# gotzmann/booster

Measured on AMD Instinct MI355X. Metric: decode tokens/sec Llama-3-8B Q4_K_M, higher is better.
Workload: dtype int8xint4/6 dot -> f32 (Q4_K/Q6_K weights x Q8_K activations), f16 KV; 1 GPU; Llama-3-8B Q4_K_M shapes (synthetic GGUF, random K-quant blocks), greedy batch-1 decode on 1xMI355X, 128-token prompt, n_ctx 2304, n_kv 133..2087; parallelism=single GPU, aql_runs=2, replay=AQL packets, fence scope NONE, own HSA queue (csrc/bamd_aql.h)

## Files before the change

### booster_amd/csrc/bamd_device.h

```cpp
#pragma once
#include <hip/hip_runtime.h>
#include <hip/hip_fp16.h>
#include <stdint.h>
#include <stdlib.h>
#include "bamd_formats.h"
#include "bamd_kernels.h"
#include "bamd_aql.h"

#define WAVE 64
#ifndef BAMD_SCHED_GROUP
#define BAMD_SCHED_GROUP 4
#endif

#ifdef BAMD_TIMING
#define TL_STAMP(tl, k) do { if ((tl) && (threadIdx.x & 63) == 0 && blockIdx.x < BAMD_TL_WG && blockIdx.y == 0) { const int w_ = (int) (threadIdx.x >> 6); \
        if (w_ == 0 || w_ == 7) (tl)[(size_t) blockIdx.x * BAMD_TL_WG_WORDS + (w_ ? 8 : 0) + (k)] = wall_clock64(); \
        if ((k) == 7 && w_ < 8) (tl)[(size_t) blockIdx.x * BAMD_TL_WG_WORDS + 16 + w_] = wall_clock64(); } } while (0)
#else
#define TL_STAMP(tl, k) do { } while (0)
#endif

__device__ __forceinline__ float h2f(uint32_t bits16) { return __half2float(__ushort_as_half((unsigned short) bits16)); }
__device__ __forceinline__ unsigned short f2h(float f) { return __half_as_ushort(__float2half_rn(f)); }
__device__ __forceinline__ int sdot4(uint32_t a, uint32_t b) { return __builtin_amdgcn_sdot4((int) a, (int) b, 0, false); }
// ... 117 lines not shown
    return __hiloint2double(__builtin_amdgcn_readlane(__double2hiint(v), lane), __builtin_amdgcn_readlane(__double2loint(v), lane));
}
__device__ __forceinline__ double wave_sum_f64(double s) {
    s += dpp_d<DPP_XOR1>(s); s += dpp_d<DPP_XOR2>(s); s += dpp_d<DPP_HALF_MIRROR>(s); s += dpp_d<DPP_MIRROR>(s);
    return ((readlane_d(s, 15) + readlane_d(s, 31)) + readlane_d(s, 47)) + readlane_d(s, 63);
}

#define BAMD_F64_GUARD_ULPS(n) (2 * (n) + 8)
__device__ __forceinline__ bool f32_rounding_safe(double v, int ulps) {
#ifdef BAMD_NO_F64_GUARD
    return true;
#endif
    if (v == 0.0) return true;
    const uint32_t hi = (uint32_t) __double2hiint(v), lo = (uint32_t) __double2loint(v);
    const uint32_t ex = (hi >> 20) & 0x7ffu;
    const int dist = (int) (lo & 0x1fffffffu) - 0x10000000;
    return ex >= 1023u - 126u && ex <= 1023u + 127u && (dist < 0 ? -dist : dist) > ulps;
}
__device__ __forceinline__ double seq_expsum8(const float * vals, int n) {
    double s = 0.0;
    for (int i = 0; i < n; i += 8) {
        const float a0 = vals[i] + vals[i + 4], a1 = vals[i + 1] + vals[i + 5], a2 = vals[i + 2] + vals[i + 6], a3 = vals[i + 3] + vals[i + 7];
        const float b0 = a0 + a2, b1 = a1 + a3;
        s += (double) (b0 + b1);
    }
    return s;
}

#define BAMD_ACT_BATCH 4
#ifndef BAMD_CEILING
#define BAMD_CEILING 0
#endif
#define BAMD_ACT_RED_OFF(nb) ((((size_t) (nb) * (256 + 32 + 4)) + 15) & ~(size_t) 15)
template <bool NORM>
struct ActPro {
    float4 v[BAMD_ACT_BATCH], w[BAMD_ACT_BATCH];
    int okmask;
    unsigned long long * tl = nullptr;

    template <int NB = BAMD_ACT_BATCH, int NWV = 0>
    __device__ __forceinline__ void issue(const float * __restrict__ x, const float * __restrict__ nw, int K, int i0, int bstride = 0, int blimit = 0) {
        const int lane = threadIdx.x & 63;
        if (bstride == 0) { bstride = NWV ? NWV : (int) (blockDim.x >> 6); blimit = K >> 8; }
        okmask = 0;
        const bamd_ik_rsrc rx = ik_rsrc(x);
#pragma unroll
        for (int b = 0; b < NB; ++b) {
            const int i = i0 + b * bstride;
            const bool ok = i < blimit;
            okmask |= ok ? 1 << b : 0;
            const int ic = ok ? i : blimit - 1;
            v[b] = ik_ld128f(rx, (uint32_t) lane * 16u, ic * 1024);
            if (NORM) w[b] = *(const float4 *) (nw + ic * 256 + lane * 4);
        }
    }

    template <int NB = BAMD_ACT_BATCH, int NWV = 0>
    __device__ __forceinline__ void quantize_batch(float scale, int K, int i0, uint32_t * q8, int * S, float * yd, int bstride = 0, int blimit = 0) {
        const int lane = threadIdx.x & 63;
        const int nwaves = bstride ? bstride : NWV ? NWV : (int) (blockDim.x >> 6), nb = bstride ? blimit : (K >> 8);
#if BAMD_CEILING & 1
#pragma unroll
        for (int b = 0; b < NB; ++b) {
            const int i = i0 + b * nwaves;
            if (i < nb) {
                const uint32_t packed = __float_as_uint(v[b].x) ^ (__float_as_uint(v[b].y) >> 8);
                q8[i * 64 + (lane & 7) * 8 + (lane >> 3)] = packed;
                if ((lane & 7) == 0) S[i * 8 + (lane >> 3)] = (int) (packed & 0xff);
                if (lane == 0) yd[i] = scale;
            }
        }
        return;
#endif
        uint32_t amaxb[NB];
#pragma unroll
        for (int b = 0; b < NB; ++b) {
            if (NORM) {
                v[b].x = (v[b].x * scale) * w[b].x; v[b].y = (v[b].y * scale) * w[b].y;
                v[b].z = (v[b].z * scale) * w[b].z; v[b].w = (v[b].w * scale) * w[b].w;
            }
            const float a = fmaxf(fmaxf(fmaxf(fabsf(v[b].x), fabsf(v[b].y)), fabsf(v[b].z)), fabsf(v[b].w));
            amaxb[b] = __float_as_uint(a);
        }
        uint32_t t[NB], wmax[NB];
#pragma unroll
        for (int b = 0; b < NB; ++b) t[b] = umax_(amaxb[b], (uint32_t) dpp_z<DPP_XOR1>((int) amaxb[b]));
#pragma unroll
        for (int b = 0; b < NB; ++b) t[b] = umax_(t[b], (uint32_t) dpp_z<DPP_XOR2>((int) t[b]));
#pragma unroll
        for (int b = 0; b < NB; ++b) t[b] = umax_(t[b], (uint32_t) dpp_z<DPP_HALF_MIRROR>((int) t[b]));
#pragma unroll
        for (int b = 0; b < NB; ++b) t[b] = umax_(t[b], (uint32_t) dpp_z<DPP_MIRROR>((int) t[b]));
#pragma unroll
        for (int b = 0; b < NB; ++b) t[b] = umax_(t[b], (uint32_t) __builtin_amdgcn_update_dpp(0, (int) t[b], 0x142, 0xa, 0xf, false));
#pragma unroll
        for (int b = 0; b < NB; ++b) t[b] = umax_(t[b], (uint32_t) __builtin_amdgcn_update_dpp(0, (int) t[b], 0x143, 0xc, 0xf, false));
#pragma unroll
        for (int b = 0; b < NB; ++b) wmax[b] = (uint32_t) __builtin_amdgcn_readlane((int) t[b], 63);
        float mine[NB];
#pragma unroll
        for (int b = 0; b < NB; ++b) {
            const float M = __uint_as_float(wmax[b]);
            const bool ex = fabsf(v[b].x) == M, ey = fabsf(v[b].y) == M, ez = fabsf(v[b].z) == M;
            float m = v[b].w;
            m = ez ? v[b].z : m; m = ey ? v[b].y : m; m = ex ? v[b].x : m;
            mine[b] = m;
        }
        int mxv = __float_as_int(1.0f);
#pragma unroll
        for (int b = 0; b < NB; ++b) {
            const unsigned long long who = __ballot(amaxb[b] == wmax[b]);
            const int first = __ffsll((long long) who) - 1;
            const int mxb = __builtin_amdgcn_readlane(__float_as_int(mine[b]), first);
            mxv = lane == b ? mxb : mxv;
        }
        const float isc = -127.f / __int_as_float(mxv);
        const float dd = 1.0f / isc;
#pragma unroll
        for (int b = 0; b < NB; ++b) {
            const int i = i0 + b * nwaves;
            if (i < nb) {
                const float iscale = __int_as_float(__builtin_amdgcn_readlane(__float_as_int(isc), b));
                const float d = __int_as_float(__builtin_amdgcn_readlane(__float_as_int(dd), b));
                const bool nz = wmax[b] != 0u;
                const float t0 = iscale * v[b].x + 12582912.f, t1 = iscale * v[b].y + 12582912.f;
                const float t2 = iscale * v[b].z + 12582912.f, t3 = iscale * v[b].w + 12582912.f;
                const uint32_t p01 = __builtin_amdgcn_perm(__float_as_uint(t1), __float_as_uint(t0), 0x0c0c0400u);
                const uint32_t p23 = __builtin_amdgcn_perm(__float_as_uint(t3), __float_as_uint(t2), 0x0c0c0400u);
                uint32_t packed = __builtin_amdgcn_perm(p23, p01, 0x05040100u);
                packed = nz ? packed : 0u;
                const int s4 = group8_sum(sdot4(packed, 0x01010101u));
                q8[i * 64 + (lane & 7) * 8 + (lane >> 3)] = packed;
                if ((lane & 7) == 0) S[i * 8 + (lane >> 3)] = s4;
                if (lane == 0) yd[i] = nz ? d : 0.f;
            }
        }
    }

    struct NoMid { __device__ __forceinline__ void operator()() const { } };
    template <bool SMALLK = false, typename MID = NoMid, int NB = BAMD_ACT_BATCH, int NWV = 0>
    __device__ __forceinline__ void finish(const float * __restrict__ x, const float * __restrict__ nw, float eps, int K,
                                           uint32_t * q8, int * S, float * yd, double * red, MID mid = MID()) {
        const int lane = threadIdx.x & 63, wave = wave_id(), nwaves = NWV ? NWV : (int) (blockDim.x >> 6), nb = K >> 8;
        const int step = nwaves * BAMD_ACT_BATCH;
        float scale = 1.0f;
#if BAMD_CEILING & 1
        if (NORM) { mid(); } else
#endif
        if (NORM) {
            double s = 0.0;
#pragma unroll
            for (int b = 0; b < NB; ++b) {
                if (okmask >> b & 1) { s += (double) (v[b].x * v[b].x); s += (double) (v[b].y * v[b].y); s += (double) (v[b].z * v[b].z); s += (double) (v[b].w * v[b].w); }
            }
            if (!SMALLK) for (int i0 = wave + step; i0 < nb; i0 += step) {
                ActPro<NORM> t; t.issue(x, nw, K, i0);
#pragma unroll
                for (int b = 0; b < BAMD_ACT_BATCH; ++b) {
                    if (t.okmask >> b & 1) { s += (double) (t.v[b].x * t.v[b].x); s += (double) (t.v[b].y * t.v[b].y); s += (double) (t.v[b].z * t.v[b].z); s += (double) (t.v[b].w * t.v[b].w); }
                }
            }
            s = wave_sum_f64(s);
            if (lane == 0) red[wave] = s;
            TL_STAMP(tl, 5);
            __syncthreads();
            mid();
            double tot = 0.0;
            for (int w2 = 0; w2 < nwaves; ++w2) tot += red[w2];
            double md = (K & (K - 1)) == 0 ? tot * (1.0 / (double) K) : tot / (double) K;
            float mean = (float) md;
            if (!f32_rounding_safe(md, BAMD_F64_GUARD_ULPS(K))) {
                __syncthreads();
                if (threadIdx.x == 0) {
                    double sq = 0.0;
                    for (int i = 0; i < K; ++i) { const float xv = ik_ld(x + i); sq += (double) (xv * xv); }
                    red[0] = sq;
                }
                __syncthreads();
                md = red[0] / (double) K;
                mean = (float) md;
            }
            scale = 1.0f / sqrtf(mean + eps);
        } else mid();
        quantize_batch<NB, NWV>(scale, K, wave, q8, S, yd);
        if (!SMALLK) for (int i0 = wave + step; i0 < nb; i0 += step) {
            ActPro<NORM> t; t.issue(x, nw, K, i0);
            t.quantize_batch(scale, K, i0, q8, S, yd);
        }
        TL_STAMP(tl, 6);
        __syncthreads();
    }
};

struct RowAcc { float acc, accm; };

struct RecQ4K { uint4 qs, hd; uint32_t mn47; };
struct RecQ5K { uint4 qs, hd; uint32_t qh, mn47; };
struct RecQ6K { uint4 ql; uint2 qh, sc; uint32_t d; };
struct RecQ3K { uint2 qs; uint32_t hm, sc0, sc1, sc2, d; };
struct RecQ2K { uint2 qs; uint4 sc; uint32_t dd; };

__device__ __forceinline__ void pin(uint32_t & x) { asm volatile("" : "+v"(x)); }
__device__ __forceinline__ void pin(uint2 & x) { pin(x.x); pin(x.y); }
__device__ __forceinline__ void pin(uint4 & x) { pin(x.x); pin(x.y); pin(x.z); pin(x.w); }
#if BAMD_XSCALES
__device__ __forceinline__ void pin_rec(RecQ4K & R) { pin(R.qs); pin(R.hd); pin(R.mn47); }
__device__ __forceinline__ void pin_rec(RecQ5K & R) { pin(R.qs); pin(R.hd); pin(R.qh); pin(R.mn47); }
#else
__device__ __forceinline__ void pin_rec(RecQ4K & R) { pin(R.qs); pin(R.hd); }
__device__ __forceinline__ void pin_rec(RecQ5K & R) { pin(R.qs); pin(R.hd); pin(R.qh); }
#endif
__device__ __forceinline__ void pin_rec(RecQ6K & R) { pin(R.ql); pin(R.qh); pin(R.sc); pin(R.d); }
__device__ __forceinline__ void pin_rec(RecQ3K & R) { pin(R.qs); pin(R.hm); pin(R.sc0); pin(R.sc1); pin(R.sc2); pin(R.d); }
__device__ __forceinline__ void pin_rec(RecQ2K & R) { pin(R.qs); pin(R.sc); pin(R.dd); }

typedef uint32_t u32x4_t __attribute__((ext_vector_type(4)));
typedef uint32_t u32x2_t __attribute__((ext_vector_type(2)));
// ... 39 lines not shown
    R.mn47 = 0u;
#endif
}
__device__ __forceinline__ void load_rec(RecQ5K & R, bamd_rsrc rs, int soff, int lane) {
    const uint32_t l = (uint32_t) lane;
    R.qs = bl128(rs, l * 16u, soff);
    R.qh = bl32(rs, 1024u + l * 4u, soff);
    R.hd = bl128(rs, 1280u + (l >> 3) * 16u, soff);
#if BAMD_XSCALES
    R.mn47 = bl32(rs, 1408u + (l >> 3) * 4u, soff);
#else
    R.mn47 = 0u;
#endif
}
__device__ __forceinline__ void load_rec(RecQ6K & R, bamd_rsrc rs, int soff, int lane) {
    const uint32_t l = (uint32_t) lane;
    R.ql = bl128(rs, l * 16u, soff);
    R.qh = bl64(rs, 1024u + l * 8u, soff);
    R.sc = bl64(rs, 1536u + (l >> 3) * 16u + ((l >> 2) & 1u) * 8u, soff);
    R.d  = bl16(rs, 1664u + (l >> 3) * 2u, soff);
}
__device__ __forceinline__ void load_rec(RecQ3K & R, bamd_rsrc rs, int soff, int lane) {
    const uint32_t l = (uint32_t) lane;
    R.qs = bl64(rs, l * 8u, soff);
    R.hm = bl32(rs, 512u + l * 4u, soff);
    R.sc0 = bl32(rs, 768u + (l >> 3) * 12u, soff); R.sc1 = bl32(rs, 772u + (l >> 3) * 12u, soff); R.sc2 = bl32(rs, 776u + (l >> 3) * 12u, soff);
    R.d  = bl16(rs, 864u + (l >> 3) * 2u, soff);
}
__device__ __forceinline__ void load_rec(RecQ2K & R, bamd_rsrc rs, int soff, int lane) {
    const uint32_t l = (uint32_t) lane;
    R.qs = bl64(rs, l * 8u, soff);
    R.sc = bl128(rs, 512u + (l >> 3) * 16u, soff);
    R.dd = bl32(rs, 640u + (l >> 3) * 4u, soff);
}
__device__ __forceinline__ void unpack_k4(const uint4 & hd, uint32_t & sc03, uint32_t & sc47, uint32_t & mn03, uint32_t & mn47) {
    const uint32_t u0 = hd.y, u1 = hd.z, u2 = hd.w;
    sc03 = u0 & 0x3f3f3f3fu; mn03 = u1 & 0x3f3f3f3fu;
    sc47 = (u2 & 0x0f0f0f0fu) | (((u0 >> 6) & 0x03030303u) << 4);
    mn47 = ((u2 >> 4) & 0x0f0f0f0fu) | (((u1 >> 6) & 0x03030303u) << 4);
}
#define BYTE(w, k) (int) (((w) >> (8 * (k))) & 0xffu)

struct Terms { float d, fs, dmin, pm; };

__device__ __forceinline__ Terms block_terms(const RecQ4K & R, int ci, int lane, const uint32_t * q8, const int * S, const float * yd) {
    const int e = lane & 7, l = e & 3;
    const float ydv = yd[ci];
    Terms T;
    T.d = ydv * h2f(R.hd.x & 0xffffu);
    T.dmin = (-ydv) * h2f(R.hd.x >> 16);
#if BAMD_XSCALES
    const uint32_t sc03 = R.hd.y, sc47 = R.hd.z, mn03 = R.hd.w, mn47 = R.mn47;
#else
    uint32_t sc03, sc47, mn03, mn47; unpack_k4(R.hd, sc03, sc47, mn03, mn47);
#endif
    const uint4 a0 = *(const uint4 *) (q8 + ci * 64 + e * 8), a1 = *(const uint4 *) (q8 + ci * 64 + e * 8 + 4);
    const uint32_t wq[8] = { R.qs.x & 0x0f0f0f0fu, (R.qs.x >> 4) & 0x0f0f0f0fu, R.qs.y & 0x0f0f0f0fu, (R.qs.y >> 4) & 0x0f0f0f0fu,
                             R.qs.z & 0x0f0f0f0fu, (R.qs.z >> 4) & 0x0f0f0f0fu, R.qs.w & 0x0f0f0f0fu, (R.qs.w >> 4) & 0x0f0f0f0fu };
    const uint32_t aq[8] = { a0.x, a0.y, a0.z, a0.w, a1.x, a1.y, a1.z, a1.w };
    const int sumi = dotscale8<false>(wq, aq, sc03, sc47);
    T.fs = (float) sumi;
    const uint32_t mw = (l < 2) ? mn03 : mn47;
    const int sh = (l & 1) * 16;
    const int ma = (int) ((mw >> sh) & 0xffu), mb = (int) ((mw >> (sh + 8)) & 0xffu);
    const int2 sp = *(const int2 *) (S + ci * 8 + 2 * l);
    T.pm = (float) (mul24(ma, sp.x) + mul24(mb, sp.y));
// ... 491 lines not shown
```

### booster_amd/csrc/bamd_matvec_core.h

```cpp
#pragma once
#include "bamd_device.h"
#include "bamd_mv_select.h"

template <int TYPE> struct RecOf;
template <> struct RecOf<BAMD_Q4_K> { typedef RecQ4K type; };
template <> struct RecOf<BAMD_Q5_K> { typedef RecQ5K type; };
template <> struct RecOf<BAMD_Q6_K> { typedef RecQ6K type; };
template <> struct RecOf<BAMD_Q3_K> { typedef RecQ3K type; };
template <> struct RecOf<BAMD_Q2_K> { typedef RecQ2K type; };

#define BAMD_NB1(NBW_) ((NBW_) < BAMD_ACT_BATCH ? (NBW_) : BAMD_ACT_BATCH)
#define BAMD_NB2(NBW_) ((NBW_) > BAMD_ACT_BATCH ? (NBW_) - BAMD_ACT_BATCH : 1)
#define BAMD_LEAD_PARAMS const float * x_, const float * nw_, const void * w0_, const void * w1_, int K_, float eps_
#define BAMD_LEAD_TAKE(a_) do { (a_).x = x_; (a_).normw = nw_; (a_).seg[0].w = w0_; (a_).seg[1].w = w1_; (a_).K = K_; (a_).eps = eps_; } while (0)
#define BAMD_LEAD_ARGS(a_) (a_).x, (a_).normw, (a_).seg[0].w, (a_).seg[1].w, (a_).K, (a_).eps
__device__ __forceinline__ ProArgs carve_lds(const bamd_mv_args & a, unsigned char * smem) {
    const int nb = a.K >> 8;
    ProArgs pa;
    pa.x = a.x; pa.nw = a.normw; pa.eps = a.eps; pa.K = a.K;
    pa.q8 = (uint32_t *) smem; pa.S = (int *) (pa.q8 + nb * 64); pa.yd = (float *) (pa.S + nb * 8);
    pa.tl = a.tl;
    pa.red = (double *) (smem + BAMD_ACT_RED_OFF(nb));
    return pa;
}


#define BAMD_EPI_HALF_GATE 16
#define BAMD_EPI_HALF_UP 17
template <int TYPE, int D, int EPI, int PRO, bool SMALLK = false, int NBP = BAMD_ACT_BATCH>
__device__ __forceinline__ void stream_segment(const uint8_t * __restrict__ wA, const uint8_t * __restrict__ wB, int nb,
                                               int first, int count, int stride, float * __restrict__ out,
                                               const float * __restrict__ res, const ProArgs & pa, ActPro<PRO == BAMD_PRO_NORM> & ap,
                                               bool issue_here, bool do_pro, unsigned long long & best, int nvalid, float * half_slot = nullptr, int * half_flag = nullptr) {
    typedef typename RecOf<TYPE>::type REC;
    constexpr int RECB = BAMD_RECB_OF(TYPE); static_assert(RECB > 0, "no wave-stream record for this type");
    constexpr bool PAIR = EPI == BAMD_EPI_SILU_MUL;
    constexpr int NPARTS = PAIR ? 2 : 1;
    const int lane = threadIdx.x & 63;
    const bamd_rsrc rsA = weight_rsrc(wA), rsB = PAIR ? weight_rsrc(wB) : rsA, rsN = null_rsrc(wA);
    const int rgb = nb * RECB;
    const int rg_step = stride * rgb;
    const int chunks = nb / D;
    if (issue_here) BAMD_PRO_ISSUE(ap, pa);
    REC ring[D];
    const int offA = count > 0 ? first * rgb : 0;
    const int fill_step = count > 0 ? RECB : 0;
#ifndef BAMD_RING_SPLIT
#define BAMD_RING_SPLIT 1
#endif
    constexpr bool RSPLIT = BAMD_RING_SPLIT && SMALLK && PRO == BAMD_PRO_NORM;
#pragma unroll
    for (int s = 0; s < (RSPLIT ? D / 2 : D); ++s) load_rec(ring[s], rsA, offA + s * fill_step, lane);
    TL_STAMP(pa.tl, 1);
    if (do_pro) {
        if (RSPLIT) {
            auto second_half = [&]() {
#pragma unroll
                for (int s = D / 2; s < D; ++s) load_rec(ring[s], rsA, offA + s * fill_step, lane);
            };
            BAMD_PRO_FINISH_NB_MID(ap, pa, second_half, NBP, 0);
        } else if (SMALLK) { auto nm = []() { }; BAMD_PRO_FINISH_NB_MID(ap, pa, nm, NBP, 0); }
        else BAMD_PRO_FINISH(ap, pa);
    } else if (RSPLIT) {
#pragma unroll
        for (int s = D / 2; s < D; ++s) load_rec(ring[s], rsA, offA + s * fill_step, lane);
    }
    TL_STAMP(pa.tl, 2);
    const uint32_t * q8 = pa.q8; const int * S = pa.S; const float * yd = pa.yd;
    for (int r = 0; r < count; ++r) {
        const int rg = first + r * stride;
        const int row = rg * 8 + (lane >> 3);
        const int rowoff = rg * rgb;
        float gate_val = 0.f;
#pragma unroll
        for (int part = 0; part < NPARTS; ++part) {
            const bool last = !(PAIR && part == 0) && r + 1 >= count;
            const bool after_b = (PAIR && part == 0) || (last && part == 1);
            const int after_off = (PAIR && part == 0) ? rowoff : (last ? rowoff + (nb - 1) * RECB : rowoff + rg_step);
            float resv = 0.f;
            if (EPI == BAMD_EPI_ADD && row < nvalid) resv = ik_ld(res + row);
            RowAcc A = { 0.f, 0.f };
            for (int c = 0; c < chunks; ++c) {
                const bool inrow = c + 1 < chunks;
                const bool tail = !inrow && last;
                const bamd_rsrc nrs = tail ? rsN : (inrow ? part == 1 : after_b) ? rsB : rsA;
                const int nxt = inrow ? rowoff + (c + 1) * (D * RECB) : after_off;
                const int step = (inrow || !last) ? RECB : 0;
#pragma unroll
                for (int s = 0; s < D; ++s) {
                    pin_rec(ring[s]);
                    const Terms T = block_terms(ring[s], c * D + s, lane, q8, S, yd);
                    chain_step<TYPE>(A, T.d, T.fs, T.dmin, T.pm);
                    load_rec(ring[s], nrs, nxt + s * step, lane);
                    if ((s & (BAMD_SCHED_GROUP - 1)) == BAMD_SCHED_GROUP - 1)
// ... 18 lines not shown
            } else if ((lane & 7) == 0 && row < nvalid) {
                float o = val;
                if (EPI == BAMD_EPI_ADD) o = val + resv;
                ik_st(out + row, o);
                if (EPI == BAMD_EPI_ARGMAX) { const unsigned long long k = argmax_key(o, row); best = k > best ? k : best; }
            }
        }
    }
}


template <int TYPE> __device__ __forceinline__ void hold_acc(RowAcc & A) {
    asm volatile("" : "+v"(A.acc));
    if (TYPE == BAMD_Q4_K || TYPE == BAMD_Q5_K) asm volatile("" : "+v"(A.accm));
}

template <int TYPE, int NBP, bool HELPER>
__device__ __forceinline__ void stream_pair_short(const uint8_t * __restrict__ wG, const uint8_t * __restrict__ wU, int rg0, int rg_stride, int j,
                                                  float * __restrict__ out, const ProArgs & pa, ActPro<true> & ap, float4 * park, int * flags, int nvalid) {
    typedef typename RecOf<TYPE>::type REC;
    constexpr int RECB = BAMD_RECB_OF(TYPE); static_assert(RECB > 0, "no wave-stream record for this type");
    constexpr int NB = 16, Q = NB / 4, CUT = NB - Q, D = 8, NREC = HELPER ? 3 * 2 * Q : 2 * CUT;
    static_assert(NREC % D == 0, "whole ring chunks");
    const int lane = threadIdx.x & 63;
    const bamd_rsrc rsG = weight_rsrc(wG), rsU = weight_rsrc(wU);
    const int rgb = NB * RECB;
#define BAMD_GU7_UP(i_)  (HELPER ? (((i_) % (2 * Q)) / Q) == 1 : ((i_) / CUT) == 1)
#define BAMD_GU7_SB(i_)  (HELPER ? CUT + ((i_) % Q) : (i_) % CUT)
#define BAMD_GU7_OFF(i_) ((HELPER ? rg0 + ((i_) / (2 * Q)) * rg_stride : rg0) * rgb + BAMD_GU7_SB(i_) * RECB)
    REC ring[D];
#pragma unroll
    for (int s = 0; s < D / 2; ++s) load_rec(ring[s], BAMD_GU7_UP(s) ? rsU : rsG, BAMD_GU7_OFF(s), lane);
    TL_STAMP(pa.tl, 1);
    auto second_half = [&]() {
#pragma unroll
        for (int s = D / 2; s < D; ++s) load_rec(ring[s], BAMD_GU7_UP(s) ? rsU : rsG, BAMD_GU7_OFF(s), lane);
    };
    BAMD_PRO_FINISH_NB_MID(ap, pa, second_half, NBP, 0);
    TL_STAMP(pa.tl, 2);
    const uint32_t * q8 = pa.q8; const int * S = pa.S; const float * yd = pa.yd;
    RowAcc Ag = { 0.f, 0.f }, Au = { 0.f, 0.f };
#pragma unroll
    for (int c = 0; c < NREC / D; ++c) {
#pragma unroll
        for (int s = 0; s < D; ++s) {
            const int i = c * D + s;
            pin_rec(ring[s]);
            const Terms T = block_terms(ring[s], BAMD_GU7_SB(i), lane, q8, S, yd);
            if (HELPER) park[((i / (2 * Q)) * 2 + (BAMD_GU7_UP(i) ? 1 : 0)) * Q * 64 + (i % Q) * 64 + lane] = make_float4(T.d, T.fs, T.dmin, T.pm);
            else if (BAMD_GU7_UP(i)) chain_step<TYPE>(Au, T.d, T.fs, T.dmin, T.pm);
            else chain_step<TYPE>(Ag, T.d, T.fs, T.dmin, T.pm);
            if (i + D < NREC) load_rec(ring[s], BAMD_GU7_UP(i + D) ? rsU : rsG, BAMD_GU7_OFF(i + D), lane);
            if (HELPER && (i % Q) == Q - 1) {
                __builtin_amdgcn_fence(__ATOMIC_RELEASE, "workgroup");
                if (lane == 0) __hip_atomic_store(flags + i / (2 * Q), (i % (2 * Q)) + 1, __ATOMIC_RELAXED, __HIP_MEMORY_SCOPE_WORKGROUP);
            }
            if ((s & (BAMD_SCHED_GROUP - 1)) == BAMD_SCHED_GROUP - 1) __builtin_amdgcn_sched_barrier(0);
        }
        if (c == 0) TL_STAMP(pa.tl, 3);
    }
    TL_STAMP(pa.tl, 4);
    if (!HELPER) {
        hold_acc<TYPE>(Ag); hold_acc<TYPE>(Au);
        const float4 * Pg = park + (j * 2 + 0) * Q * 64 + lane, * Pu = park + (j * 2 + 1) * Q * 64 + lane;
        auto wait_for = [&](const int need) {
            while (__hip_atomic_load(flags + j, __ATOMIC_RELAXED, __HIP_MEMORY_SCOPE_WORKGROUP) < need) __builtin_amdgcn_s_sleep(1);
            __builtin_amdgcn_fence(__ATOMIC_ACQUIRE, "workgroup");
        };
        float4 tg[Q], tu[Q];
        wait_for(Q);
#pragma unroll
// ... 43 lines not shown
    }
    int bbase = first * rgb + i0 * RECB;
    REC ring[D];
#ifndef BAMD_RING_SPLIT_B
#define BAMD_RING_SPLIT_B 1
#endif
#ifndef BAMD_RING_SPLIT_MIN
#define BAMD_RING_SPLIT_MIN 6
#endif
    constexpr bool RSPLIT = BAMD_RING_SPLIT_B && SMALLK && !UNEVEN && D >= BAMD_RING_SPLIT_MIN;
    constexpr int DH = RSPLIT ? D / 2 : D;
    auto ring_fill = [&](const int s0, const int s1) {
#pragma unroll
        for (int m = 0; m < M; ++m) {
            if (SMALLK || m < count) {
#pragma unroll
                for (int j = 0; j < NBW; ++j) {
                    const int sl = m * NBW + j;
                    if (sl >= s0 && sl < s1) load_rec(ring[sl], rs, bbase + m * rg_step + (UNEVEN && j >= n_w ? n_w - 1 : j) * RECB, lane);
                }
            }
        }
    };
    ring_fill(0, DH);
    TL_STAMP(pa.tl, 1);
    pre();
    if (do_pro) {
        if (OWN) {
            static_assert(NBW <= 2 * BAMD_ACT_BATCH, "own-slice prologue handles two batches");
            ap.template quantize_batch<BAMD_NB1(NBW)>(1.0f, pa.K, i0, pa.q8, pa.S, pa.yd, 1, i0 + n_w);
            if (RSPLIT) ring_fill(DH, D);
            if (NBW > BAMD_ACT_BATCH) ap2.template quantize_batch<BAMD_NB2(NBW)>(1.0f, pa.K, i0 + BAMD_ACT_BATCH, pa.q8, pa.S, pa.yd, 1, i0 + n_w);
        } else if (SMALLK && !UNEVEN) {
            auto second_half = [&]() { if (RSPLIT) ring_fill(DH, D); };
            BAMD_PRO_FINISH_NB_MID(ap, pa, second_half, BAMD_NB1(NBW), NWV);
        }
        else if (SMALLK) BAMD_PRO_FINISH_SMALLK(ap, pa);
        else BAMD_PRO_FINISH(ap, pa);
    } else if (RSPLIT) ring_fill(DH, D);
    TL_STAMP(pa.tl, 2);
    const uint32_t * q8 = pa.q8; const int * S = pa.S; const float * yd = pa.yd;
    for (int r0 = 0; r0 < (ONEB ? 1 : count); r0 += M) {
        const int nbatch = ONEB ? M : (count - r0 < M ? count - r0 : M);
        float * B0 = part0 + (NBUF == 2 ? (size_t) (batchctr & 1) * M * rg_floats : (size_t) 0);
        const int crow = (first + (r0 + (wave < nbatch ? wave : 0)) * stride) * 8 + r8;
        float resv = 0.f;
        if (EPI == BAMD_EPI_ADD && crow < nvalid) resv = ik_ld(res + crow);
#pragma unroll
        for (int m = 0; m < M; ++m) {
            if (m < nbatch) {
                float * Pf = B0 + (size_t) m * rg_floats;
                float4 * P = (float4 *) Pf;
#pragma unroll
                for (int j = 0; j < NBW; ++j) {
                    const int s = m * NBW + j;
                    const int ci = i0 + j;
                    pin_rec(ring[s]);
                    if (!UNEVEN || j < n_w) {
                        const Terms T = block_terms(ring[s], ci, lane, q8, S, yd);
                        if (COMPACT) {
                            float * rec = Pf + (size_t) ci * 144;
                            *(float2 *) (rec + lane * 2) = make_float2(T.fs, T.pm);
                            if ((lane & 7) == 0) *(float2 *) (rec + 128 + r8 * 2) = make_float2(T.d, T.dmin);
                        } else P[ci * 64 + lane] = make_float4(T.d, T.fs, T.dmin, T.pm);
                    }
#ifndef BAMD_SPLIT_UNCOND_REFILL
#define BAMD_SPLIT_UNCOND_REFILL 1
// ... 66 lines not shown
```

### booster_amd/csrc/bamd_matvec_fast_a.hip

```cpp
#include "bamd_matvec_core.h"

template <int TYPE0, int TYPE1, int PRO, int EPI, int NBP>
__global__ void __launch_bounds__(512) matvec_fast_kernel(BAMD_LEAD_PARAMS, bamd_mv_args a) {
    BAMD_LEAD_TAKE(a);
    extern __shared__ __attribute__((aligned(16))) unsigned char smem[];
    TL_STAMP(a.tl, 0);
    const int nb = a.K >> 8;
    const ProArgs pa = carve_lds(a, smem);
    ActPro<PRO == BAMD_PRO_NORM> ap;
    BAMD_PRO_ISSUE_NB(ap, pa, NBP, 0);
    const int wave = wave_id(), nwaves = blockDim.x >> 6;
    const int slot = blockIdx.x + gridDim.x * wave;
    const int stride = gridDim.x * nwaves;
    unsigned long long best = 0ull;
    constexpr bool PAIR = EPI == BAMD_EPI_SILU_MUL;
    const int nrg0 = a.seg[0].nrows >> 3;
    const int nv0 = a.seg[0].nvalid > 0 ? a.seg[0].nvalid : a.seg[0].nrows;
    if (TYPE1 == 0) {
        const int count = a.cnt_q + (slot < a.cnt_r ? 1 : 0);
        const uint8_t * wA = (const uint8_t *) a.seg[0].w;
        const uint8_t * wB = PAIR ? (const uint8_t *) a.seg[1].w : wA;
        stream_segment<TYPE0, 8, EPI, PRO, true, NBP>(wA, wB, nb, slot, count, stride, a.seg[0].out, a.res, pa, ap, false, true, best, nv0);
    } else {
        constexpr int T1 = TYPE1 == 0 ? TYPE0 : TYPE1;
        const int nrg1 = a.seg[1].nrows >> 3;
        const int nv1 = a.seg[1].nvalid > 0 ? a.seg[1].nvalid : a.seg[1].nrows;
        if (slot >= nrg0 && slot < nrg0 + nrg1) {
            const uint8_t * w1 = (const uint8_t *) a.seg[1].w;
            stream_segment<T1, 8, EPI, PRO, true, NBP>(w1, w1, nb, slot - nrg0, 1, stride, a.seg[1].out, a.res, pa, ap, false, true, best, nv1);
        } else {
            const uint8_t * w0 = (const uint8_t *) a.seg[0].w;
            stream_segment<TYPE0, 8, EPI, PRO, true, NBP>(w0, w0, nb, slot, slot < nrg0 ? 1 : 0, stride, a.seg[0].out, a.res, pa, ap, false, true, best, nv0);
        }
    }
    if (EPI == BAMD_EPI_ARGMAX) {
        for (int o = 32; o; o >>= 1) { const unsigned long long ob = __shfl_xor(best, o); best = ob > best ? ob : best; }
        __syncthreads();
        unsigned long long * wb = (unsigned long long *) smem;
        if ((threadIdx.x & 63) == 0) wb[wave] = best;
        __syncthreads();
        if (threadIdx.x == 0) {
            unsigned long long b = 0ull;
            for (int w = 0; w < nwaves; ++w) b = wb[w] > b ? wb[w] : b;
            if (b) atomicMax(a.best_key, b);
        }
    }
    TL_STAMP(a.tl, 7);
}

template <int TYPE, int NBP>
__global__ void __launch_bounds__(512) matvec_gateup7_kernel(BAMD_LEAD_PARAMS, bamd_mv_args a) {
    BAMD_LEAD_TAKE(a);
    extern __shared__ __attribute__((aligned(16))) unsigned char smem[];
    TL_STAMP(a.tl, 0);
    const int nb = a.K >> 8;
    const ProArgs pa = carve_lds(a, smem);
    ActPro<true> ap;
    BAMD_PRO_ISSUE_NB(ap, pa, NBP, 0);
    const int wave = wave_id(), grid = (int) gridDim.x, b = (int) blockIdx.x;
    float4 * park = (float4 *) (smem + mv_park_off(nb));
    int * flags = (int *) (smem + mv_park_off(nb) + mv_gu7_park_bytes(16));
    if (threadIdx.x < 4) flags[threadIdx.x] = 0;
    const uint8_t * wG = (const uint8_t *) a.seg[0].w, * wU = (const uint8_t *) a.seg[1].w;
    const int nv = a.seg[0].nvalid > 0 ? a.seg[0].nvalid : a.seg[0].nrows;
    unsigned long long best = 0ull;
    if (wave < 4) stream_segment<TYPE, 8, BAMD_EPI_SILU_MUL, BAMD_PRO_NORM, true, NBP>(wG, wU, nb, b + grid * wave, 1, grid * 8, a.seg[0].out, a.res, pa, ap, false, true, best, nv);
    else if (wave < 7) stream_pair_short<TYPE, NBP, false>(wG, wU, b + grid * wave, grid, wave - 4, a.seg[0].out, pa, ap, park, flags, nv);
    else stream_pair_short<TYPE, NBP, true>(wG, wU, b + grid * 4, grid, 0, a.seg[0].out, pa, ap, park, flags, nv);
    TL_STAMP(a.tl, 7);
}
static const bool g_gateup7 = env_flag("BAMD_GATEUP7", true);

template <int TYPE, int NBP>
__global__ void __launch_bounds__(512) matvec_gateup14_kernel(BAMD_LEAD_PARAMS, bamd_mv_args a) {
    BAMD_LEAD_TAKE(a);
    extern __shared__ __attribute__((aligned(16))) unsigned char smem[];
    TL_STAMP(a.tl, 0);
    const int nb = a.K >> 8;
    const ProArgs pa = carve_lds(a, smem);
    ActPro<true> ap;
    BAMD_PRO_ISSUE_NB(ap, pa, NBP, 0);
    const int wave = wave_id(), grid = (int) gridDim.x, b = (int) blockIdx.x;
    float * slots = (float *) (smem + mv_park_off(nb));
    int * flags = (int *) (slots + 16);
    if (threadIdx.x < 2) flags[threadIdx.x] = 0;
    const uint8_t * wG = (const uint8_t *) a.seg[0].w, * wU = (const uint8_t *) a.seg[1].w;
    const int nv = a.seg[0].nvalid > 0 ? a.seg[0].nvalid : a.seg[0].nrows;
    unsigned long long best = 0ull;
    if (wave < 4) stream_segment<TYPE, 8, BAMD_EPI_SILU_MUL, BAMD_PRO_NORM, true, NBP>(wG, wU, nb, b + grid * wave, 2, grid * 4, a.seg[0].out, a.res, pa, ap, false, true, best, nv);
    else {
        stream_segment<TYPE, 8, BAMD_EPI_SILU_MUL, BAMD_PRO_NORM, true, NBP>(wG, wU, nb, b + grid * (4 + wave), 1, grid, a.seg[0].out, a.res, pa, ap, false, true, best, nv);
        const int h = (wave - 4) >> 1;
        const int rg = b + grid * (12 + h);
        if (((wave - 4) & 1) == 0) stream_segment<TYPE, 8, BAMD_EPI_HALF_GATE, BAMD_PRO_NORM, true, NBP>(wG, wG, nb, rg, 1, grid, a.seg[0].out, a.res, pa, ap, false, false, best, nv, slots + 8 * h, flags + h);
        else                       stream_segment<TYPE, 8, BAMD_EPI_HALF_UP, BAMD_PRO_NORM, true, NBP>(wU, wU, nb, rg, 1, grid, a.seg[0].out, a.res, pa, ap, false, false, best, nv, slots + 8 * h, flags + h);
    }
    TL_STAMP(a.tl, 7);
}
static const bool g_gateup14 = env_flag("BAMD_GATEUP14", true);

template <int PRO, int EPI, int T0, int T1>
static void launch_fast_a_inst(const bamd_mv_args & a, int grid, hipStream_t s) {
    if ((a.K >> 8) <= 16) BAMD_LAUNCH((matvec_fast_kernel<T0, T1, PRO, EPI, 2>), dim3(grid), dim3(512), act_lds_bytes(a.K), s, BAMD_LEAD_ARGS(a), a);
    else                  BAMD_LAUNCH((matvec_fast_kernel<T0, T1, PRO, EPI, 4>), dim3(grid), dim3(512), act_lds_bytes(a.K), s, BAMD_LEAD_ARGS(a), a);
}
typedef pairs<cpair<BAMD_Q4_K, BAMD_Q5_K>, cpair<BAMD_Q4_K, BAMD_Q6_K>, cpair<BAMD_Q5_K, BAMD_Q4_K>, cpair<BAMD_Q5_K, BAMD_Q6_K>, cpair<BAMD_Q6_K, BAMD_Q4_K>,
              cpair<BAMD_Q6_K, BAMD_Q5_K>, cpair<BAMD_Q2_K, BAMD_Q3_K>> fast_a_pairs;
template <int PRO, int EPI>
static bool launch_fast_a_types(const bamd_mv_args & a, int t0, int t1, int grid, hipStream_t s) {
    if (t1 == 0) return with_kquant(t0, [&](auto T) -> bool { launch_fast_a_inst<PRO, EPI, decltype(T)::value, 0>(a, grid, s); return true; });
    if constexpr (PRO == BAMD_PRO_NORM && EPI == BAMD_EPI_STORE)
        return with_pair(fast_a_pairs(), t0, t1, [&](auto P) -> bool { launch_fast_a_inst<PRO, EPI, decltype(P)::a, decltype(P)::b>(a, grid, s); return true; });
    return false;
}
// ... 23 lines not shown
```

Baseline: 686.9 tokens/s.

## Interleave second-half ring weight loads across RMSnorm/quantize prologue stages

Splits the second half of the weight-record ring prefetch into per-field load parts and spreads them over named stage points in the activation norm and quantize prologue: the DPP reduction steps, the barrier, mean, scale, max reductions and the divide. Scheduling barriers pin each group of loads at its stage. The aim is to overlap weight memory issue with the prologue's latency-bound reduction chain instead of issuing all loads in one burst at the barrier. It also makes the wave count a compile-time constant (8) for the fast_a kernels. This costs more code complexity and register pressure, and it assumes 512-thread blocks.

```diff
diff --git a/booster_amd/csrc/bamd_device.h b/booster_amd/csrc/bamd_device.h
--- a/booster_amd/csrc/bamd_device.h
+++ b/booster_amd/csrc/bamd_device.h
@@ -173,6 +173,35 @@
 #define BAMD_CEILING 0
 #endif
 #define BAMD_ACT_RED_OFF(nb) ((((size_t) (nb) * (256 + 32 + 4)) + 15) & ~(size_t) 15)
+template <int N> struct StageC { static constexpr int value = N; };
+template <int LO, int HI, typename F> __device__ __forceinline__ void static_for(F && f) {
+    if constexpr (LO < HI) { f(StageC<LO>()); static_for<LO + 1, HI>(f); }
+}
+enum {
+    BAMD_ST_SQ = 0,
+    BAMD_ST_SQ1,
+    BAMD_ST_SQ2, BAMD_ST_SQ3, BAMD_ST_SQ4,
+    BAMD_ST_BAR,
+    BAMD_ST_RED,
+    BAMD_ST_MEAN,
+    BAMD_ST_SCALE,
+    BAMD_ST_NORM,
+    BAMD_ST_MAX1,
+    BAMD_ST_MAX2, BAMD_ST_MAX3, BAMD_ST_MAX4, BAMD_ST_MAX5, BAMD_ST_MAX6,
+    BAMD_ST_FIRST,
+    BAMD_ST_DIV,
+    BAMD_ST_END,
+    BAMD_ST_COUNT
+};
+template <typename MID, typename = void> struct MidStaged { static constexpr bool value = false; };
+template <typename MID> struct MidStaged<MID, decltype((*(MID *) nullptr)(StageC<0>()), void())> { static constexpr bool value = true; };
+template <int ST, typename MID> __device__ __forceinline__ void mid_at(MID & mid, int) {
+    if constexpr (MidStaged<MID>::value) mid(StageC<ST>());
+    else if constexpr (ST == BAMD_ST_BAR) mid();
+}
+template <int LO, int HI, typename MID> __device__ __forceinline__ void mid_span(MID & mid) {
+    static_for<LO, HI>([&](auto st) { mid_at<decltype(st)::value>(mid, 0); });
+}
 template <bool NORM>
 struct ActPro {
     float4 v[BAMD_ACT_BATCH], w[BAMD_ACT_BATCH];
@@ -196,11 +225,13 @@
         }
     }
 
-    template <int NB = BAMD_ACT_BATCH, int NWV = 0>
-    __device__ __forceinline__ void quantize_batch(float scale, int K, int i0, uint32_t * q8, int * S, float * yd, int bstride = 0, int blimit = 0) {
+    struct NoMid { __device__ __forceinline__ void operator()() const { } };
+    template <int NB = BAMD_ACT_BATCH, int NWV = 0, typename MID = NoMid>
+    __device__ __forceinline__ void quantize_batch(float scale, int K, int i0, uint32_t * q8, int * S, float * yd, int bstride = 0, int blimit = 0, MID mid = MID()) {
         const int lane = threadIdx.x & 63;
         const int nwaves = bstride ? bstride : NWV ? NWV : (int) (blockDim.x >> 6), nb = bstride ? blimit : (K >> 8);
 #if BAMD_CEILING & 1
+        mid_span<BAMD_ST_NORM, BAMD_ST_DIV + 1>(mid);
 #pragma unroll
         for (int b = 0; b < NB; ++b) {
             const int i = i0 + b * nwaves;
@@ -223,19 +254,26 @@
             const float a = fmaxf(fmaxf(fmaxf(fabsf(v[b].x), fabsf(v[b].y)), fabsf(v[b].z)), fabsf(v[b].w));
             amaxb[b] = __float_as_uint(a);
         }
+        mid_at<BAMD_ST_NORM>(mid, 0);
         uint32_t t[NB], wmax[NB];
 #pragma unroll
         for (int b = 0; b < NB; ++b) t[b] = umax_(amaxb[b], (uint32_t) dpp_z<DPP_XOR1>((int) amaxb[b]));
+        mid_at<BAMD_ST_MAX1>(mid, 0);
 #pragma unroll
         for (int b = 0; b < NB; ++b) t[b] = umax_(t[b], (uint32_t) dpp_z<DPP_XOR2>((int) t[b]));
+        mid_at<BAMD_ST_MAX2>(mid, 0);
 #pragma unroll
         for (int b = 0; b < NB; ++b) t[b] = umax_(t[b], (uint32_t) dpp_z<DPP_HALF_MIRROR>((int) t[b]));
+        mid_at<BAMD_ST_MAX3>(mid, 0);
 #pragma unroll
         for (int b = 0; b < NB; ++b) t[b] = umax_(t[b], (uint32_t) dpp_z<DPP_MIRROR>((int) t[b]));
+        mid_at<BAMD_ST_MAX4>(mid, 0);
 #pragma unroll
         for (int b = 0; b < NB; ++b) t[b] = umax_(t[b], (uint32_t) __builtin_amdgcn_update_dpp(0, (int) t[b], 0x142, 0xa, 0xf, false));
+        mid_at<BAMD_ST_MAX5>(mid, 0);
 #pragma unroll
         for (int b = 0; b < NB; ++b) t[b] = umax_(t[b], (uint32_t) __builtin_amdgcn_update_dpp(0, (int) t[b], 0x143, 0xc, 0xf, false));
+        mid_at<BAMD_ST_MAX6>(mid, 0);
 #pragma unroll
         for (int b = 0; b < NB; ++b) wmax[b] = (uint32_t) __builtin_amdgcn_readlane((int) t[b], 63);
         float mine[NB];
@@ -255,8 +293,10 @@
             const int mxb = __builtin_amdgcn_readlane(__float_as_int(mine[b]), first);
             mxv = lane == b ? mxb : mxv;
         }
+        mid_at<BAMD_ST_FIRST>(mid, 0);
         const float isc = -127.f / __int_as_float(mxv);
         const float dd = 1.0f / isc;
+        mid_at<BAMD_ST_DIV>(mid, 0);
 #pragma unroll
         for (int b = 0; b < NB; ++b) {
             const int i = i0 + b * nwaves;
@@ -278,7 +318,6 @@
         }
     }
 
-    struct NoMid { __device__ __forceinline__ void operator()() const { } };
     template <bool SMALLK = false, typename MID = NoMid, int NB = BAMD_ACT_BATCH, int NWV = 0>
     __device__ __forceinline__ void finish(const float * __restrict__ x, const float * __restrict__ nw, float eps, int K,
                                            uint32_t * q8, int * S, float * yd, double * red, MID mid = MID()) {
@@ -286,7 +325,7 @@
         const int step = nwaves * BAMD_ACT_BATCH;
         float scale = 1.0f;
 #if BAMD_CEILING & 1
-        if (NORM) { mid(); } else
+        if (NORM) { if constexpr (MidStaged<MID>::value) mid_span<BAMD_ST_SQ, BAMD_ST_SCALE + 1>(mid); else mid(); } else
 #endif
         if (NORM) {
             double s = 0.0;
@@ -301,13 +340,21 @@
                     if (t.okmask >> b & 1) { s += (double) (t.v[b].x * t.v[b].x); s += (double) (t.v[b].y * t.v[b].y); s += (double) (t.v[b].z * t.v[b].z); s += (double) (t.v[b].w * t.v[b].w); }
                 }
             }
-            s = wave_sum_f64(s);
+            if constexpr (MidStaged<MID>::value) {
+                mid_at<BAMD_ST_SQ>(mid, 0);
+                s += dpp_d<DPP_XOR1>(s);        mid_at<BAMD_ST_SQ1>(mid, 0);
+                s += dpp_d<DPP_XOR2>(s);        mid_at<BAMD_ST_SQ2>(mid, 0);
+                s += dpp_d<DPP_HALF_MIRROR>(s); mid_at<BAMD_ST_SQ3>(mid, 0);
+                s += dpp_d<DPP_MIRROR>(s);      mid_at<BAMD_ST_SQ4>(mid, 0);
+                s = ((readlane_d(s, 15) + readlane_d(s, 31)) + readlane_d(s, 47)) + readlane_d(s, 63);
+            } else s = wave_sum_f64(s);
             if (lane == 0) red[wave] = s;
             TL_STAMP(tl, 5);
             __syncthreads();
-            mid();
+            if constexpr (MidStaged<MID>::value) mid_at<BAMD_ST_BAR>(mid, 0); else mid();
             double tot = 0.0;
             for (int w2 = 0; w2 < nwaves; ++w2) tot += red[w2];
+            mid_at<BAMD_ST_RED>(mid, 0);
             double md = (K & (K - 1)) == 0 ? tot * (1.0 / (double) K) : tot / (double) K;
             float mean = (float) md;
             if (!f32_rounding_safe(md, BAMD_F64_GUARD_ULPS(K))) {
@@ -321,9 +368,14 @@
                 md = red[0] / (double) K;
                 mean = (float) md;
             }
+            mid_at<BAMD_ST_MEAN>(mid, 0);
             scale = 1.0f / sqrtf(mean + eps);
-        } else mid();
-        quantize_batch<NB, NWV>(scale, K, wave, q8, S, yd);
+            mid_at<BAMD_ST_SCALE>(mid, 0);
+        } else if constexpr (MidStaged<MID>::value) mid_span<BAMD_ST_SQ, BAMD_ST_SCALE + 1>(mid);
+        else mid();
+        if constexpr (MidStaged<MID>::value) quantize_batch<NB, NWV, MID &>(scale, K, wave, q8, S, yd, 0, 0, mid);
+        else quantize_batch<NB, NWV>(scale, K, wave, q8, S, yd);
+        mid_at<BAMD_ST_END>(mid, 0);
         if (!SMALLK) for (int i0 = wave + step; i0 < nb; i0 += step) {
             ActPro<NORM> t; t.issue(x, nw, K, i0);
             t.quantize_batch(scale, K, i0, q8, S, yd);
@@ -429,6 +481,55 @@
     R.qs = bl64(rs, l * 8u, soff);
     R.sc = bl128(rs, 512u + (l >> 3) * 16u, soff);
     R.dd = bl32(rs, 640u + (l >> 3) * 4u, soff);
+}
+template <typename REC> struct RecLoads;
+template <> struct RecLoads<RecQ4K> { static constexpr int value = BAMD_XSCALES ? 3 : 2; };
+template <> struct RecLoads<RecQ5K> { static constexpr int value = BAMD_XSCALES ? 4 : 3; };
+template <> struct RecLoads<RecQ6K> { static constexpr int value = 4; };
+template <> struct RecLoads<RecQ3K> { static constexpr int value = 6; };
+template <> struct RecLoads<RecQ2K> { static constexpr int value = 3; };
+template <int P> __device__ __forceinline__ void load_rec_part(RecQ4K & R, bamd_rsrc rs, int soff, int lane) {
+    const uint32_t l = (uint32_t) lane;
+    if (P == 0) R.qs = bl128(rs, l * 16u, soff);
+    if (P == 1) R.hd = bl128(rs, 1024u + (l >> 3) * 16u, soff);
+#if BAMD_XSCALES
+    if (P == 2) R.mn47 = bl32(rs, 1152u + (l >> 3) * 4u, soff);
+#else
+    if (P == 1) R.mn47 = 0u;
+#endif
+}
+template <int P> __device__ __forceinline__ void load_rec_part(RecQ5K & R, bamd_rsrc rs, int soff, int lane) {
+    const uint32_t l = (uint32_t) lane;
+    if (P == 0) R.qs = bl128(rs, l * 16u, soff);
+    if (P == 1) R.qh = bl32(rs, 1024u + l * 4u, soff);
+    if (P == 2) R.hd = bl128(rs, 1280u + (l >> 3) * 16u, soff);
+#if BAMD_XSCALES
+    if (P == 3) R.mn47 = bl32(rs, 1408u + (l >> 3) * 4u, soff);
+#else
+    if (P == 2) R.mn47 = 0u;
+#endif
+}
+template <int P> __device__ __forceinline__ void load_rec_part(RecQ6K & R, bamd_rsrc rs, int soff, int lane) {
+    const uint32_t l = (uint32_t) lane;
+    if (P == 0) R.ql = bl128(rs, l * 16u, soff);
+    if (P == 1) R.qh = bl64(rs, 1024u + l * 8u, soff);
+    if (P == 2) R.sc = bl64(rs, 1536u + (l >> 3) * 16u + ((l >> 2) & 1u) * 8u, soff);
+    if (P == 3) R.d  = bl16(rs, 1664u + (l >> 3) * 2u, soff);
+}
+template <int P> __device__ __forceinline__ void load_rec_part(RecQ3K & R, bamd_rsrc rs, int soff, int lane) {
+    const uint32_t l = (uint32_t) lane;
+    if (P == 0) R.qs = bl64(rs, l * 8u, soff);
+    if (P == 1) R.hm = bl32(rs, 512u + l * 4u, soff);
+    if (P == 2) R.sc0 = bl32(rs, 768u + (l >> 3) * 12u, soff);
+    if (P == 3) R.sc1 = bl32(rs, 772u + (l >> 3) * 12u, soff);
+    if (P == 4) R.sc2 = bl32(rs, 776u + (l >> 3) * 12u, soff);
+    if (P == 5) R.d  = bl16(rs, 864u + (l >> 3) * 2u, soff);
+}
+template <int P> __device__ __forceinline__ void load_rec_part(RecQ2K & R, bamd_rsrc rs, int soff, int lane) {
+    const uint32_t l = (uint32_t) lane;
+    if (P == 0) R.qs = bl64(rs, l * 8u, soff);
+    if (P == 1) R.sc = bl128(rs, 512u + (l >> 3) * 16u, soff);
+    if (P == 2) R.dd = bl32(rs, 640u + (l >> 3) * 4u, soff);
 }
 __device__ __forceinline__ void unpack_k4(const uint4 & hd, uint32_t & sc03, uint32_t & sc47, uint32_t & mn03, uint32_t & mn47) {
     const uint32_t u0 = hd.y, u1 = hd.z, u2 = hd.w;
diff --git a/booster_amd/csrc/bamd_matvec_core.h b/booster_amd/csrc/bamd_matvec_core.h
--- a/booster_amd/csrc/bamd_matvec_core.h
+++ b/booster_amd/csrc/bamd_matvec_core.h
@@ -24,6 +24,29 @@
     return pa;
 }
 
+
+#ifndef BAMD_RING_DRIP
+#define BAMD_RING_DRIP 1
+#endif
+#ifndef BAMD_RING_DRIP_B
+#define BAMD_RING_DRIP_B 0
+#endif
+#ifndef BAMD_PRO_NWV_A
+#define BAMD_PRO_NWV_A 8
+#endif
+template <int MODE, int ST, int NL, typename ONE> __device__ __forceinline__ void drip_stage(ONE && one) {
+    constexpr int FIRST = MODE == 2 ? BAMD_ST_SQ1 : MODE == 3 ? BAMD_ST_END : BAMD_ST_BAR, LAST = MODE == 3 ? BAMD_ST_END : BAMD_ST_DIV;
+    constexpr int NS = LAST - FIRST + 1, PER = (NL + NS - 1) / NS, k = ST - FIRST;
+    static_assert(NS >= 1 && PER * NS >= NL, "every request has a stage point");
+    if constexpr (k >= 0 && k < NS) {
+        constexpr int lo = k * PER < NL ? k * PER : NL, hi = (k + 1) * PER < NL ? (k + 1) * PER : NL;
+        if constexpr (lo < hi) {
+            __builtin_amdgcn_sched_barrier(0);
+            static_for<lo, hi>(one);
+            __builtin_amdgcn_sched_barrier(0);
+        }
+    }
+}
 
 #define BAMD_EPI_HALF_GATE 16
 #define BAMD_EPI_HALF_UP 17
@@ -54,12 +77,22 @@
     TL_STAMP(pa.tl, 1);
     if (do_pro) {
         if (RSPLIT) {
+#if BAMD_RING_DRIP
+            constexpr int LPR = RecLoads<REC>::value;
+            auto second_half = [&](auto st) {
+                drip_stage<BAMD_RING_DRIP, decltype(st)::value, (D - D / 2) * LPR>([&](auto n) {
+                    constexpr int s = D / 2 + decltype(n)::value / LPR;
+                    load_rec_part<decltype(n)::value % LPR>(ring[s], rsA, offA + s * fill_step, lane);
+                });
+            };
+#else
             auto second_half = [&]() {
 #pragma unroll
                 for (int s = D / 2; s < D; ++s) load_rec(ring[s], rsA, offA + s * fill_step, lane);
             };
-            BAMD_PRO_FINISH_NB_MID(ap, pa, second_half, NBP, 0);
-        } else if (SMALLK) { auto nm = []() { }; BAMD_PRO_FINISH_NB_MID(ap, pa, nm, NBP, 0); }
+#endif
+            BAMD_PRO_FINISH_NB_MID(ap, pa, second_half, NBP, BAMD_PRO_NWV_A);
+        } else if (SMALLK) { auto nm = []() { }; BAMD_PRO_FINISH_NB_MID(ap, pa, nm, NBP, BAMD_PRO_NWV_A); }
         else BAMD_PRO_FINISH(ap, pa);
     } else if (RSPLIT) {
 #pragma unroll
@@ -144,11 +177,21 @@
 #pragma unroll
     for (int s = 0; s < D / 2; ++s) load_rec(ring[s], BAMD_GU7_UP(s) ? rsU : rsG, BAMD_GU7_OFF(s), lane);
     TL_STAMP(pa.tl, 1);
+#if BAMD_RING_DRIP
+    constexpr int LPR = RecLoads<REC>::value;
+    auto second_half = [&](auto st) {
+        drip_stage<BAMD_RING_DRIP, decltype(st)::value, (D - D / 2) * LPR>([&](auto n) {
+            constexpr int s = D / 2 + decltype(n)::value / LPR;
+            load_rec_part<decltype(n)::value % LPR>(ring[s], BAMD_GU7_UP(s) ? rsU : rsG, BAMD_GU7_OFF(s), lane);
+        });
+    };
+#else
     auto second_half = [&]() {
 #pragma unroll
         for (int s = D / 2; s < D; ++s) load_rec(ring[s], BAMD_GU7_UP(s) ? rsU : rsG, BAMD_GU7_OFF(s), lane);
     };
-    BAMD_PRO_FINISH_NB_MID(ap, pa, second_half, NBP, 0);
+#endif
+    BAMD_PRO_FINISH_NB_MID(ap, pa, second_half, NBP, BAMD_PRO_NWV_A);
     TL_STAMP(pa.tl, 2);
     const uint32_t * q8 = pa.q8; const int * S = pa.S; const float * yd = pa.yd;
     RowAcc Ag = { 0.f, 0.f }, Au = { 0.f, 0.f };
@@ -258,7 +301,17 @@
             if (RSPLIT) ring_fill(DH, D);
             if (NBW > BAMD_ACT_BATCH) ap2.template quantize_batch<BAMD_NB2(NBW)>(1.0f, pa.K, i0 + BAMD_ACT_BATCH, pa.q8, pa.S, pa.yd, 1, i0 + n_w);
         } else if (SMALLK && !UNEVEN) {
+#if BAMD_RING_DRIP_B
+            constexpr int LPR = RecLoads<REC>::value;
+            auto second_half = [&](auto st) {
+                if constexpr (RSPLIT) drip_stage<BAMD_RING_DRIP_B, decltype(st)::value, (D - DH) * LPR>([&](auto n) {
+                    constexpr int sl = DH + decltype(n)::value / LPR;
+                    load_rec_part<decltype(n)::value % LPR>(ring[sl], rs, bbase + (sl / NBW) * rg_step + (sl % NBW) * RECB, lane);
+                });
+            };
+#else
             auto second_half = [&]() { if (RSPLIT) ring_fill(DH, D); };
+#endif
             BAMD_PRO_FINISH_NB_MID(ap, pa, second_half, BAMD_NB1(NBW), NWV);
         }
         else if (SMALLK) BAMD_PRO_FINISH_SMALLK(ap, pa);
diff --git a/booster_amd/csrc/bamd_matvec_fast_a.hip b/booster_amd/csrc/bamd_matvec_fast_a.hip
--- a/booster_amd/csrc/bamd_matvec_fast_a.hip
+++ b/booster_amd/csrc/bamd_matvec_fast_a.hip
@@ -8,7 +8,7 @@
     const int nb = a.K >> 8;
     const ProArgs pa = carve_lds(a, smem);
     ActPro<PRO == BAMD_PRO_NORM> ap;
-    BAMD_PRO_ISSUE_NB(ap, pa, NBP, 0);
+    BAMD_PRO_ISSUE_NB(ap, pa, NBP, BAMD_PRO_NWV_A);
     const int wave = wave_id(), nwaves = blockDim.x >> 6;
     const int slot = blockIdx.x + gridDim.x * wave;
     const int stride = gridDim.x * nwaves;
@@ -56,7 +56,7 @@
     const int nb = a.K >> 8;
     const ProArgs pa = carve_lds(a, smem);
     ActPro<true> ap;
-    BAMD_PRO_ISSUE_NB(ap, pa, NBP, 0);
+    BAMD_PRO_ISSUE_NB(ap, pa, NBP, BAMD_PRO_NWV_A);
     const int wave = wave_id(), grid = (int) gridDim.x, b = (int) blockIdx.x;
     float4 * park = (float4 *) (smem + mv_park_off(nb));
     int * flags = (int *) (smem + mv_park_off(nb) + mv_gu7_park_bytes(16));
@@ -79,7 +79,7 @@
     const int nb = a.K >> 8;
     const ProArgs pa = carve_lds(a, smem);
     ActPro<true> ap;
-    BAMD_PRO_ISSUE_NB(ap, pa, NBP, 0);
+    BAMD_PRO_ISSUE_NB(ap, pa, NBP, BAMD_PRO_NWV_A);
     const int wave = wave_id(), grid = (int) gridDim.x, b = (int) blockIdx.x;
     float * slots = (float *) (smem + mv_park_off(nb));
     int * flags = (int *) (slots + 16);
```

After: 694.8 tokens/s (median of 6 runs). 1.01x the previous value.
